# rgcgithub/regenie

Hardware: AMD Instinct MI355X
Metric: Step-1 SNPs x samples x phenos / sec (higher is better)
Workload: dtype fp4 (exact integer Gram) + i8 (exact fixed-point digit planes of the fp64 operands: G~X / G~Y, many-row predictions) + f64 (solves, level 1); 1 GPU; BASELINE configs[1]: synthetic PLINK bed 50000 samples x 100000 SNPs (100000 per GPU), 1 QT pheno, bsize 1000, 22 chromosomes, 5-fold CV, 5x5 ridge grid; `value` is the HBM-resident figure (packed genotypes generated on the device, timed region = level 0 + level 1 + LOCO rows); the complete run from files on disk is `end_to_end_from_files`; samples=50000, snps=100000, phenos=1, bsize=1000, blocks=109, parallelism=blocks sharded x1, all-gather of W, level-1 Gram tiles / ridge systems shared x1

## Files before the change

regenie_amd/build.py:

```python
from __future__ import annotations

import concurrent.futures as cf
import hashlib
import os
import shutil
import subprocess
import sys

HERE = os.path.dirname(os.path.abspath(__file__))
CSRC = os.path.join(HERE, "csrc")
LIBDIR = os.path.join(HERE, "lib")
LIB = os.path.join(LIBDIR, "librg_step1_hip.so")
SOURCES = ["rg_api.hip", "bed_prep.hip", "gram_i8.hip", "gram_fp4.hip", "assemble.hip", "chol.hip", "pred.hip", "l1.hip", "ubench.hip", "loocv.hip", "loocv_tri.hip", "l1x.hip", "l0_f64.hip", "step2_qt.hip", "step2_bt.hip", "step2_mcc.hip", "rg_group.hip", "pred_i8.hip", "xy_i8.hip", "wgram_bf16.hip", "bgen_inflate.hip", "ld_corr.hip",
           "pgen_api.cpp", "bgen_api.cpp"]
HOST_SOURCES = ["driver_common.cpp", "driver_models.cpp", "driver_inputs.cpp", "driver_step2.cpp", "driver_step2_bgen.cpp", "driver_ld.cpp", "driver_step1.cpp", "driver_main.cpp"]
FLAGS = ["--offload-arch=gfx950", "-O3", "-std=c++17", "-fPIC", "-Wall", "-Wno-unused-function",
         "-Wno-unused-variable", "-Wno-unused-value", "-Wno-unused-result", "-Wno-inline-asm"]


def _hipcc() -> str:
    for c in (shutil.which("hipcc"), "/opt/rocm/bin/hipcc"):
        if c and os.path.exists(c):
            return c
    raise RuntimeError("hipcc not found")
# ... 24 lines not shown
        with open(os.path.join(HERE, rel), "rb") as fh:
            out[rel] = hashlib.sha256(fh.read()).hexdigest()
    out["flags"] = hashlib.sha256(" ".join(FLAGS).encode()).hexdigest()
    return out


def _deps():
    return _lib_deps() + [os.path.join(HERE, "host", f) for f in HOST_SOURCES + ["driver.h", "driver_step2.h", "driver_ld.h", "fmt_g6.h"]]


def _lib_deps():
    return [os.path.join(CSRC, s) for s in SOURCES] + [
                                                      os.path.join(CSRC, "rg_internal.h"),
                                                      os.path.join(CSRC, "chol_common.h"),
                                                      os.path.join(CSRC, "chol_p128.h"),
                                                      os.path.join(CSRC, "step2_internal.h"),
                                                      os.path.join(CSRC, "pgen_reader.h"),
                                                      os.path.join(CSRC, "bgen_reader.h"),
                                                      os.path.join(CSRC, "inflate_fast.h"),
                                                      os.path.join(HERE, "..", "include", "rg_bgen.h"),
                                                      os.path.join(HERE, "..", "include", "rg_ld.h"),
                                                      os.path.join(HERE, "..", "include", "rg_pgen.h"),
                                                      os.path.join(HERE, "..", "include", "rg_step1.h"),
                                                      os.path.join(HERE, "..", "include", "rg_step2.h")]


def _write_file_digests():
    import json
    with open(os.path.join(LIBDIR, "kernel_files.json"), "w") as fh:
        json.dump(kernel_file_digests(), fh, indent=0, sort_keys=True)
# ... 60 lines not shown
```

regenie_amd/csrc/l1.hip:

```cpp
#include <algorithm>
#include <climits>
#include <cmath>
#include <cstdint>
#include <vector>
#include "rg_internal.h"

#define CT 64

struct L1Rows {
  const double* W; const double* y; const double* zero;
  int64_t Np; int L, P, p, n64;
};
__device__ __forceinline__ const double* l1_row(const L1Rows& R, int row) {
  if (row < R.L) return R.W + ((int64_t)row * R.P + R.p) * R.Np;
  if (row == R.n64) return R.y;
  return R.zero;
}

struct L1G64 {
  L1Rows R; int T, rtot, nslice, ntile, world, rank;
  double* out; int64_t slice_stride;
};
__global__ __launch_bounds__(256, 2) void k_l1_gram64(L1G64 g, SegLayout seg) {
  const int lane = threadIdx.x & 63, wave = threadIdx.x >> 6;
// ... 48 lines not shown
        mma8(a0, b0);
        if (kc + 2 < k1) load8(a0, b0, kc + 2);
        mma8(a1, b1);
      }
    }
  }
  double* O = g.out + (int64_t)sl * g.slice_stride + (int64_t)f * g.rtot * g.R.n64 + (int64_t)tr * CT * g.R.n64 + tc * CT;
#pragma unroll
  for (int m = 0; m < 4; ++m)
#pragma unroll
    for (int n = 0; n < 4; ++n)
#pragma unroll
      for (int r = 0; r < 4; ++r) O[(int64_t)(m * 16 + q + 4 * r) * g.R.n64 + n * 16 + i] = acc[m][n][r];
}

struct L1Item { int16_t mr, mc, fold, slice; };
struct L1G128 {
  L1Rows R; int rtot, nslice; const L1Item* items; double* out; int64_t slice_stride;
};
#define G128_STAGE 32768
__device__ __forceinline__ const double* l1_wrow(const L1Rows& R, int row) {
  return row < R.L ? R.W + ((int64_t)row * R.P + R.p) * R.Np : R.zero;
}
__global__ __launch_bounds__(256, 2) void k_l1_gram128(L1G128 g, SegLayout seg) {
  __shared__ __attribute__((aligned(16))) uint8_t smem[2 * G128_STAGE];
  const L1Item it = g.items[blockIdx.x];
  if (it.fold < 0) return;
  const int lane = threadIdx.x & 63, wave = __builtin_amdgcn_readfirstlane(threadIdx.x >> 6);
  const int wr = wave >> 1, wc = wave & 1;
  const int i = lane & 15, q = lane >> 4;
  const int f = it.fold, n64 = g.R.n64;
// ... 72 lines not shown
  const double* y = R.y + seg.pos_start[f];
  const int64_t n = seg.plen[f];
  double t0 = 0.0, t1 = 0.0;
  for (int64_t e = 2 * (int64_t)threadIdx.x; e < n; e += 512) {
    const double2 wv = *reinterpret_cast<const double2*>(w + e), yv = *reinterpret_cast<const double2*>(y + e);
    t0 = fma(wv.x, yv.x, t0);
    t1 = fma(wv.y, yv.y, t1);
  }
  double t = t0 + t1;
  for (int o = 32; o > 0; o >>= 1) t += __shfl_down(t, o);
  if ((threadIdx.x & 63) == 0) red[threadIdx.x >> 6] = t;
  __syncthreads();
  if (threadIdx.x == 0) out[(int64_t)f * rtot * R.n64 + (int64_t)R.n64 * R.n64 + l] = (red[0] + red[1]) + (red[2] + red[3]);
}

static std::vector<L1Item> l1_build_items(int n64, int K, int nslice, int world, int rank) {
  const int T2 = (n64 + 127) / 128, S = 4, TS = (T2 + S - 1) / S;
  std::vector<std::vector<L1Item>> xl(8);
  int gi = 0;
  for (int f = 0; f < K; ++f)
    for (int sl = 0; sl < nslice; ++sl)
      for (int Mr = 0; Mr < TS; ++Mr)
        for (int Mc = 0; Mc <= Mr; ++Mc) {
          std::vector<L1Item>& dst = xl[gi % 8];
          bool any = false;
          for (int mr = Mr * S; mr < std::min(T2, (Mr + 1) * S); ++mr)
            for (int mc = Mc * S; mc < std::min(T2, (Mc + 1) * S); ++mc) {
              if (mc > mr) continue;
              if ((mr * (mr + 1) / 2 + mc) % world != rank) continue;
              dst.push_back(L1Item{(int16_t)mr, (int16_t)mc, (int16_t)f, (int16_t)sl});
              any = true;
            }
          if (any) ++gi;
        }
  size_t mx = 0;
  for (auto& v : xl) mx = std::max(mx, v.size());
  std::vector<L1Item> items(mx * 8, L1Item{0, 0, -1, 0});
  for (int x = 0; x < 8; ++x)
    for (size_t j = 0; j < xl[x].size(); ++j) items[8 * j + x] = xl[x][j];
  return items;
}

void rg_launch_fold_gram_rows(hipStream_t st, const double* G, int64_t ld, int L, int n64, int rtot, const double* zero,
                              const SegLayout& seg, double* out) {
  L1G64 g;
  g.R = L1Rows{G, zero, zero, ld, L, 1, 0, n64};
  g.T = n64 / CT; g.rtot = rtot; g.nslice = 1; g.ntile = g.T * (g.T + 1) / 2 + g.T; g.world = 1; g.rank = 0;
  g.out = out; g.slice_stride = 0;
  hipLaunchKernelGGL(k_l1_gram64, dim3((g.ntile + 3) / 4, seg.nseg), dim3(256), 0, st, g, seg);
}

__global__ void k_reduce_slices(const double* part, int64_t slice_stride, int nslice, int64_t n, double* out) {
  const int64_t e = (int64_t)blockIdx.x * blockDim.x + threadIdx.x;
  if (e >= n) return;
  double t = 0.0;
  for (int s = 0; s < nslice; ++s) t += part[(int64_t)s * slice_stride + e];
  out[e] = t;
}

__global__ void k_sum_folds(const double* fold, int64_t msz, int nfold, double* sum) {
  const int64_t e = (int64_t)blockIdx.x * blockDim.x + threadIdx.x;
  if (e >= msz) return;
  double t = 0.0;
  for (int f = 0; f < nfold; ++f) t += fold[(int64_t)f * msz + e];
  sum[e] = t;
}

__global__ __launch_bounds__(256) void k_loco(const double* pred, int nchr, int64_t N, const int32_t* chrom, int nchrom,
                                              double* out) {
  const int64_t n = (int64_t)blockIdx.x * 256 + threadIdx.x;
  if (n >= N) return;
  double tot = 0.0;
  for (int k = 0; k < nchr; ++k) tot += pred[(int64_t)k * N + n];
  for (int c = 0; c < nchrom; ++c) out[(int64_t)c * N + n] = tot;
  for (int k = 0; k < nchr; ++k) out[(int64_t)(chrom[k] - 1) * N + n] = tot - pred[(int64_t)k * N + n];
}

int rg_emit_pred(rg_ctx* ctx, hipStream_t st, const double* d_pred, int nchr, int p, double* pred_out) {
  const int64_t N = ctx->N;
  if (ctx->loco_nchrom <= 0) {
    RG_HIP(hipMemcpyAsync(pred_out + (int64_t)p * nchr * N, d_pred, sizeof(double) * (size_t)nchr * N, hipMemcpyDeviceToHost, st));
    return RG_OK;
  }
  if ((int)ctx->loco_chrom.size() != nchr) { ctx->err = "LOCO output: rg_set_loco_output was given a different number of chromosomes"; return RG_ERR_ARG; }
  const int nchrom = ctx->loco_nchrom;
  double* d_out = (double*)rg_ws(ctx, 11, sizeof(double) * (size_t)nchrom * N + sizeof(int32_t) * (size_t)nchr + 64);
  if (!d_out) { ctx->err = "LOCO output: out of device memory"; return RG_ERR_HIP; }
  int32_t* d_chr = reinterpret_cast<int32_t*>(d_out + (size_t)nchrom * N);
  RG_HIP(hipMemcpyAsync(d_chr, ctx->loco_chrom.data(), sizeof(int32_t) * nchr, hipMemcpyHostToDevice, st));
  hipLaunchKernelGGL(k_loco, dim3((unsigned)((N + 255) / 256)), dim3(256), 0, st, d_pred, nchr, N, d_chr, nchrom, d_out);
  RG_HIP(hipMemcpyAsync(pred_out + (int64_t)p * nchrom * N, d_out, sizeof(double) * (size_t)nchrom * N, hipMemcpyDeviceToHost, st));
  return RG_OK;
}

__global__ __launch_bounds__(256) void k_tiles_pack(double* fold, int64_t msz, int T, int n64, double* packed, int unpack) {
  const int t = blockIdx.x, f = blockIdx.y;
  int tr = (int)((sqrtf(8.0f * t + 1.0f) - 1.0f) * 0.5f);
  while ((tr + 1) * (tr + 2) / 2 <= t) ++tr;
  while (tr * (tr + 1) / 2 > t) --tr;
  int tc = t - tr * (tr + 1) / 2;
  if (tr >= T) { tc = t - T * (T + 1) / 2; tr = T; }
  double* src = fold + (int64_t)f * msz + (int64_t)tr * CT * n64 + tc * CT;
  double* pk = packed + ((int64_t)f * gridDim.x + t) * (CT * CT);
  for (int e = threadIdx.x; e < CT * CT; e += 256) {
    const int r = e >> 6, c = e & 63;
    if (unpack) src[(int64_t)r * n64 + c] = pk[e];
    else pk[e] = src[(int64_t)r * n64 + c];
  }
}

#define R1MAX 8
#define L1_CT 256
__global__ __launch_bounds__(256) void k_l1_cv(L1Rows R, const double* alpha , int R1,
                                               const int32_t* chunk_seg, const int64_t* chunk_pos,
                                               const int64_t* chunk_len, double* part) {
  __shared__ double sA[L1_CT][R1MAX];
  __shared__ double sred[4][R1MAX * 3 + 2];
  const int ch = blockIdx.x;
  const int f = chunk_seg[ch];
  const int64_t p0 = chunk_pos[ch], plen = chunk_len[ch];
  double tot[R1MAX * 3 + 2];
#pragma unroll
  for (int t = 0; t < R1MAX * 3 + 2; ++t) tot[t] = 0.0;
  for (int64_t sub = 0; sub < plen; sub += 256) {
    const int64_t pos = p0 + sub + threadIdx.x;
    const bool live = sub + threadIdx.x < plen;
    double acc[R1MAX];
#pragma unroll
    for (int j = 0; j < R1MAX; ++j) acc[j] = 0.0;
    for (int c0 = 0; c0 < R.L; c0 += L1_CT) {
      __syncthreads();
      for (int j = 0; j < R1MAX; ++j) {
        const int col = c0 + threadIdx.x;
        sA[threadIdx.x][j] = (j < R1 && col < R.L)
            ? alpha[((int64_t)f * R1 + j) * R.n64 + col] : 0.0;
      }
      __syncthreads();
      if (live) {
        const int cn = min(L1_CT, R.L - c0);
        const double* w = R.W + ((int64_t)c0 * R.P + R.p) * R.Np + pos;
        for (int c = 0; c < cn; ++c) {
          const double x = w[(int64_t)c * R.P * R.Np];
#pragma unroll
          for (int j = 0; j < R1MAX; ++j) acc[j] = fma(x, sA[c][j], acc[j]);
        }
      }
    }
    if (live) {
      const double y = R.y[pos];
#pragma unroll
      for (int j = 0; j < R1MAX; ++j) {
        tot[3 * j] += acc[j];
        tot[3 * j + 1] = fma(acc[j], acc[j], tot[3 * j + 1]);
        tot[3 * j + 2] = fma(acc[j], y, tot[3 * j + 2]);
      }
      tot[R1MAX * 3] += y;
      tot[R1MAX * 3 + 1] = fma(y, y, tot[R1MAX * 3 + 1]);
    }
  }
#pragma unroll
  for (int t = 0; t < R1MAX * 3 + 2; ++t) {
    double x = tot[t];
    for (int o = 32; o > 0; o >>= 1) x += __shfl_down(x, o);
    if ((threadIdx.x & 63) == 0) sred[threadIdx.x >> 6][t] = x;
  }
  __syncthreads();
  if (threadIdx.x < R1MAX * 3 + 2)
    part[(int64_t)ch * (R1MAX * 3 + 2) + threadIdx.x] =
        (sred[0][threadIdx.x] + sred[1][threadIdx.x]) + (sred[2][threadIdx.x] + sred[3][threadIdx.x]);
}

__global__ __launch_bounds__(256) void k_l1_pred(L1Rows R, const double* alpha , int R1,
                                                 int best, const int32_t* chunk_seg,
                                                 const int64_t* chunk_pos, const int64_t* chunk_len,
                                                 const int32_t* chr_col0 , int nchr,
                                                 const int32_t* cidx, int64_t N, double* pred) {
  extern __shared__ double sAl[];
  const int ch = blockIdx.x;
  const int f = chunk_seg[ch];
  const int64_t p0 = chunk_pos[ch], plen = chunk_len[ch];
  const double* al = alpha + ((int64_t)f * R1 + best) * R.n64;
  for (int c = threadIdx.x; c < R.L; c += 256) sAl[c] = al[c];
  __syncthreads();
  for (int64_t sub = 0; sub < plen; sub += 256) {
    const int64_t pos = p0 + sub + threadIdx.x;
    if (sub + threadIdx.x >= plen) continue;
    const int32_t n = cidx[pos];
    if (n < 0) continue;
    for (int c = 0; c < nchr; ++c) {
      double acc = 0.0;
      const double* w = R.W + ((int64_t)chr_col0[c] * R.P + R.p) * R.Np + pos;
      const int nn = chr_col0[c + 1] - chr_col0[c];
      for (int t = 0; t < nn; ++t) acc = fma(w[(int64_t)t * R.P * R.Np], sAl[chr_col0[c] + t], acc);
      pred[(int64_t)c * N + n] = acc;
    }
  }
}

int rg_l1_qt_impl(rg_ctx* ctx, int R1, const double* tau, int nchr, const int32_t* cols_per_chr,
                  double* cumsum_out, int32_t* best_out, double* pred_out) {
  if (!ctx->have_problem || !(ctx->d_W || ctx->v_W)) { ctx->err = "rg_l1_qt: no level-0 predictors"; return RG_ERR_STATE; }
  if (R1 < 1 || R1 > R1MAX) { ctx->err = "rg_l1_qt: n_ridge_l1 must be in [1,8]"; return RG_ERR_ARG; }
  if (ctx->loocv) { ctx->err = "rg_l1_qt: the problem was set up for LOOCV (use rg_l1_qt_loocv)"; return RG_ERR_STATE; }
  hipStream_t st = ctx->stream;
  const int L = ctx->B_total * ctx->R0, K = ctx->K;
  if (!ctx->v_W && ctx->w_nb != ctx->B_total) { ctx->err = "rg_l1_qt: W holds a block range only (rg_set_block_range): level 1 needs the exchanged view"; return RG_ERR_STATE; }
  const double* Wv = ctx->v_W ? ctx->v_W : ctx->d_W;
  const int Pv = ctx->v_W ? ctx->v_np : ctx->P, P = ctx->v_np, p0v = ctx->v_p0;
  int ltot = 0;
  std::vector<int32_t> col0(nchr + 1, 0);
  for (int c = 0; c < nchr; ++c) { col0[c + 1] = col0[c] + cols_per_chr[c]; }
  ltot = col0[nchr];
  if (ltot != L) { ctx->err = "rg_l1_qt: cols_per_chr does not sum to n_blocks*R0"; return RG_ERR_ARG; }
  const int n64 = (int)rg_round_up(L, CT), rtot = n64 + CT, T = n64 / CT;
  const int64_t msz = (int64_t)rtot * n64;
  const int nsys = K * R1;
  const int nch = ctx->n_c256;
  const int NPART = R1MAX * 3 + 2;
  const int world = ctx->coll_world, rank = ctx->coll_rank;
  const bool multi = ctx->coll_allreduce != nullptr;
  const int b0 = multi ? (int)((int64_t)nsys * rank / world) : 0;
  const int b1 = multi ? (int)((int64_t)nsys * (rank + 1) / world) : nsys;
  const int nloc = b1 - b0;
  const int ntile = T * (T + 1) / 2 + T;
  int64_t min_nch = INT64_MAX;
  for (int f = 0; f < K; ++f) min_nch = std::min(min_nch, ctx->seg.plen[f] / 64);
  const int T2 = (n64 + 127) / 128, ntile2 = T2 * (T2 + 1) / 2;
  int nslice = (int)std::min<int64_t>(16, std::max<int64_t>(1, (3072 + (int64_t)ntile2 * K - 1) / ((int64_t)ntile2 * K)));
  nslice = (int)std::max<int64_t>(1, std::min<int64_t>(nslice, min_nch / 2));

  double *d_fold = nullptr, *d_part = nullptr, *d_sum = nullptr, *d_wk = nullptr, *d_dinv = nullptr, *d_tau = nullptr,
         *d_cvp = nullptr, *d_pred = nullptr, *d_alpha = nullptr, *d_pack = nullptr;
  int32_t* d_col0 = nullptr;
#define L1_WS(var, slot, type, count)                                                   \
  var = (type*)rg_ws(ctx, slot, sizeof(type) * (size_t)(count));                        \
  if (!var) { ctx->err = "rg_l1_qt: out of device memory"; return RG_ERR_HIP; }
  L1_WS(d_fold, 0, double, msz * K)
  if (nslice > 1) { L1_WS(d_part, 1, double, msz * K * nslice) }
  L1_WS(d_sum, 2, double, msz)
  L1_WS(d_wk, 3, double, msz * std::max(1, nloc))
  L1_WS(d_dinv, 4, double, rg_chol_ws_doubles((size_t)std::max(1, nloc), n64))
  L1_WS(d_tau, 5, double, R1)
  L1_WS(d_cvp, 6, double, (size_t)nch * NPART)
  L1_WS(d_pred, 7, double, (size_t)nchr * ctx->N)
  L1_WS(d_alpha, 8, double, (size_t)nsys * n64)
  L1_WS(d_col0, 9, int32_t, nchr + 1)
  if (multi) { L1_WS(d_pack, 10, double, (size_t)ntile * K * CT * CT) }
  L1Item* d_items = nullptr;
  const std::vector<L1Item> items = l1_build_items(n64, K, nslice, multi ? world : 1, multi ? rank : 0);
  L1_WS(d_items, 12, L1Item, items.size())
  RG_HIP(hipMemcpyAsync(d_items, items.data(), sizeof(L1Item) * items.size(), hipMemcpyHostToDevice, st));
  RG_HIP(hipStreamSynchronize(st));
#undef L1_WS
  RG_HIP(hipMemcpyAsync(d_col0, col0.data(), sizeof(int32_t) * (nchr + 1), hipMemcpyHostToDevice, st));
  std::vector<double> hpart((size_t)nch * NPART);
  int rc = RG_OK;
  auto lap = [&](double* slot, hipEvent_t e0, hipEvent_t e1) {
    if (!ctx->timing) return;
    hipEventRecord(e1, st); hipEventSynchronize(e1);
    float ms; hipEventElapsedTime(&ms, e0, e1); *slot += ms;
    hipEventRecord(e0, st);
  };

  for (int p = 0; p < P && rc == RG_OK; ++p) {
    const int pg = p0v + p, pw = ctx->v_W ? p : pg;
    L1Rows R{Wv, ctx->d_V + (int64_t)(ctx->C + pg) * ctx->Np, ctx->d_zero, ctx->Np, L, Pv, pw, n64};
    hipEvent_t e0 = ctx->ev0, e1 = ctx->ev1;
    if (ctx->timing) hipEventRecord(e0, st);
    double* gout = nslice > 1 ? d_part : d_fold;
    hipMemsetAsync(gout, 0, sizeof(double) * msz * K * nslice, st);
    L1G128 g{R, rtot, nslice, d_items, gout, msz * K};
    hipLaunchKernelGGL(k_l1_gram128, dim3((unsigned)items.size()), dim3(256), 0, st, g, ctx->seg);
    if (nslice > 1)
      hipLaunchKernelGGL(k_reduce_slices, dim3((unsigned)((msz * K + 255) / 256)), dim3(256), 0, st, d_part, msz * K,
                         nslice, msz * K, d_fold);
    hipLaunchKernelGGL(k_l1_wty, dim3(L, K), dim3(256), 0, st, R, ctx->seg, rtot, multi ? world : 1, multi ? rank : 0, d_fold);
    if (multi) {
      hipLaunchKernelGGL(k_tiles_pack, dim3(ntile, K), dim3(256), 0, st, d_fold, msz, T, n64, d_pack, 0);
      RG_HIP(hipStreamSynchronize(st));
      if (ctx->coll_allreduce(ctx->coll_user, d_pack, (int64_t)ntile * K * CT * CT) != 0) { ctx->err = "rg_l1_qt: all-reduce callback failed"; rc = RG_ERR_STATE; break; }
      hipLaunchKernelGGL(k_tiles_pack, dim3(ntile, K), dim3(256), 0, st, d_fold, msz, T, n64, d_pack, 1);
    }
    hipLaunchKernelGGL(k_sum_folds, dim3((unsigned)((msz + 255) / 256)), dim3(256), 0, st, d_fold, msz, K, d_sum);
    lap(&ctx->tm.ms_l1_gram, e0, e1);
    hipMemcpyAsync(d_tau, tau + (int64_t)p * R1, sizeof(double) * R1, hipMemcpyHostToDevice, st);
    hipMemsetAsync(d_alpha, 0, sizeof(double) * (size_t)nsys * n64, st);
    if (nloc > 0) {
      rg_launch_chol_solve_formed_x(st, d_sum, 0, d_fold, msz, K, d_tau, R1, nullptr, L, 1, d_wk, msz, n64, CT, 1,
                                    d_dinv, ctx->d_info + 1, &ctx->tm.n_chol_launches, 1, nullptr, 0, 0, 1, b0, nloc);
      RG_HIP(hipMemcpy2DAsync(d_alpha + (int64_t)b0 * n64, sizeof(double) * n64, d_wk + (int64_t)n64 * n64,
                              sizeof(double) * msz, sizeof(double) * n64, nloc, hipMemcpyDeviceToDevice, st));
    }
    if (multi) {
      RG_HIP(hipStreamSynchronize(st));
      if (ctx->coll_allreduce(ctx->coll_user, d_alpha, (int64_t)nsys * n64) != 0) { ctx->err = "rg_l1_qt: all-reduce callback failed"; rc = RG_ERR_STATE; break; }
    }
    lap(&ctx->tm.ms_l1_chol, e0, e1);
    hipLaunchKernelGGL(k_l1_cv, dim3(nch), dim3(256), 0, st, R, d_alpha, R1, ctx->d_c256_seg,
                       ctx->d_c256_pos, ctx->d_c256_len, d_cvp);
    RG_HIP(hipMemcpyAsync(hpart.data(), d_cvp, sizeof(double) * hpart.size(), hipMemcpyDeviceToHost, st));
    RG_HIP(hipStreamSynchronize(st));
    double* cs = cumsum_out + (int64_t)p * 5 * R1;
    for (int t = 0; t < 5 * R1; ++t) cs[t] = 0.0;
    double sy = 0.0, sy2 = 0.0;
    for (int ch = 0; ch < nch; ++ch) {
      const double* q = hpart.data() + (size_t)ch * NPART;
      for (int j = 0; j < R1; ++j) {
        cs[0 * R1 + j] += q[3 * j];
        cs[2 * R1 + j] += q[3 * j + 1];
        cs[4 * R1 + j] += q[3 * j + 2];
      }
      sy += q[R1MAX * 3];
      sy2 += q[R1MAX * 3 + 1];
    }
    for (int j = 0; j < R1; ++j) { cs[1 * R1 + j] = sy; cs[3 * R1 + j] = sy2; }
    int best = 0; double minv = 1e10;
    for (int j = 0; j < R1; ++j) {
      const double perf = (cs[2 * R1 + j] + cs[3 * R1 + j] - 2 * cs[4 * R1 + j]) / ctx->neff[pg];
      if (perf < minv) { best = j; minv = perf; }
    }
    best_out[p] = best;
    hipMemsetAsync(d_pred, 0, sizeof(double) * (size_t)nchr * ctx->N, st);
    hipLaunchKernelGGL(k_l1_pred, dim3(nch), dim3(256), sizeof(double) * L, st, R, d_alpha, R1, best,
                       ctx->d_c256_seg, ctx->d_c256_pos, ctx->d_c256_len, d_col0, nchr,
                       ctx->d_cidx, ctx->N, d_pred);
    if ((rc = rg_emit_pred(ctx, st, d_pred, nchr, p, pred_out))) break;
    RG_HIP(hipStreamSynchronize(st));
    if (ctx->timing) { hipEventRecord(e1, st); hipEventSynchronize(e1); float ms; hipEventElapsedTime(&ms, e0, e1); ctx->tm.ms_l1_pred += ms; }
    int32_t info[2] = {0, 0};
    RG_HIP(hipMemcpy(info, ctx->d_info, sizeof(info), hipMemcpyDeviceToHost));
    if (info[1]) { ctx->err = "level 1 ridge system is not positive definite"; rc = RG_ERR_NOT_SPD; }
  }
  return rc;
}
```

regenie_amd/csrc/rg_api.hip:

```cpp
#include <algorithm>
#include <cstdlib>
#include <cstring>
#include <chrono>
#include "rg_internal.h"

namespace {

template <class T>
int dev_alloc(rg_ctx* ctx, T** p, size_t n) {
  if (*p) { hipFree(*p); *p = nullptr; }
  if (n == 0) n = 1;
  RG_HIP(hipMalloc((void**)p, n * sizeof(T)));
  return RG_OK;
}
template <class T>
int dev_upload(rg_ctx* ctx, T** p, const std::vector<T>& v) {
  int rc = dev_alloc(ctx, p, v.size());
  if (rc) return rc;
  if (!v.empty()) RG_HIP(hipMemcpy(*p, v.data(), v.size() * sizeof(T), hipMemcpyHostToDevice));
  return RG_OK;
}

void free_all(rg_ctx* c) {
  void* ptrs[] = {c->d_cidx, c->d_act, c->d_V, c->d_maskp, c->d_Q, c->d_XtY, c->d_lambda, c->d_neff,
// ... 44 lines not shown
  hipEventCreate(&c->ev0);
  hipEventCreate(&c->ev1);
  *out = c;
  return RG_OK;
}

void rg_destroy(rg_ctx* c) {
  if (!c) return;
  hipSetDevice(c->device);
  if (c->twin) { rg_destroy(c->twin); c->twin = nullptr; }
  if (c->ev_ingest) hipEventDestroy(c->ev_ingest);
  if (c->ev_tw_fork) hipEventDestroy(c->ev_tw_fork);
  if (c->ev_tw_join) hipEventDestroy(c->ev_tw_join);
  hipStreamSynchronize(c->stream);
  free_all(c);
  if (c->ev0) hipEventDestroy(c->ev0);
  if (c->ev1) hipEventDestroy(c->ev1);
  if (c->ev_fork) {
    hipEventDestroy(c->ev_fork);
    for (int k = 0; k < 3; ++k) { hipStreamSynchronize(c->st_part[k]); hipStreamDestroy(c->st_part[k]); hipEventDestroy(c->ev_part[k]); }
  }
  if (c->st_stage) { hipStreamSynchronize(c->st_stage); hipStreamDestroy(c->st_stage); }
  if (c->own_stream) hipStreamDestroy(c->stream);
  delete c;
}

const char* rg_last_error(const rg_ctx* c) { return c ? c->err.c_str() : "null context"; }

int rg_set_problem(rg_ctx* ctx, const rg_problem* p) {
  if (!ctx || !p) return RG_ERR_ARG;
// ... 820 lines not shown
```

regenie_amd/csrc/rg_internal.h:

```cpp
#pragma once
#include <hip/hip_runtime.h>
#include <stdint.h>
#include <functional>
#include <string>
#include <vector>

#include "../../include/rg_step1.h"

#define RG_MAX_SEG 32
#define RG_TILE_G 128
#define RG_TILE_C 64

typedef int v4i __attribute__((ext_vector_type(4)));
typedef int v16i __attribute__((ext_vector_type(16)));
typedef double v4d __attribute__((ext_vector_type(4)));

static inline int64_t rg_round_up(int64_t x, int64_t m) { return (x + m - 1) / m * m; }
static inline size_t rg_chol_ws_doubles(size_t batch, int n64) {
  const size_t T = (size_t)n64 / 64;
  return batch * (T + (T + 3) / 4 * 10) * 4096;
}

struct SegLayout {
  int32_t nseg;
// ... 117 lines not shown
  rg_allreduce_fn coll_allreduce = nullptr;
  void* coll_user = nullptr;

  rg_ctx* twin = nullptr;
  int n_pipe = 1;
  bool is_child = false;
  hipEvent_t ev_tw_fork = nullptr, ev_tw_join = nullptr;
  bool join_pending = false;
  int pipe_rr = 0;

  hipEvent_t ev_ingest = nullptr;
  bool ingest_pending = false;

  void* ws_ptr[16] = {};
  size_t ws_bytes[16] = {};

  void* f64_ptr[10] = {};
  size_t f64_bytes[10] = {};

  bool timing = false;
  rg_timing tm{};
  hipEvent_t ev0 = nullptr, ev1 = nullptr;
};

static inline double* rg_w_base(const rg_ctx* c) { return c->d_W ? c->d_W - (int64_t)c->w_b0 * c->R0 * c->P * c->Np : nullptr; }

static inline void* rg_ws(rg_ctx* ctx, int slot, size_t bytes) {
  if (bytes == 0) bytes = 8;
  if (ctx->ws_bytes[slot] < bytes) {
    if (ctx->ws_ptr[slot]) hipFree(ctx->ws_ptr[slot]);
// ... 108 lines not shown
  int64_t Np, pk_ld, pk_blk_stride;
  const uint8_t* pk; const double* mu; const double* sc; const double* Bm; const double* V;
  const double* maskp; const double* neff; const int32_t* bs; const int32_t* blockid;
  const double* wk; double* gt; double* W;
  int64_t gt_pos0 = 0, gt_len = 0;
};
size_t rg_loocv_tri_ws_doubles(int nblk, int n64, int P, int R0);
int rg_l0_loocv_tri(rg_ctx* ctx, hipStream_t st, const LoocvArgs& la, int max_bs, const double* d_sum, int rtot, double* ws, double* zt,
                    int64_t chunk, const std::function<void(int64_t, int64_t)>& gt_chunk);
void rg_launch_decode_gt(hipStream_t st, const LoocvArgs& a);
void rg_launch_l0_loocv(hipStream_t st, const LoocvArgs& a, double* part0, double* part1, int nchunk);
void rg_launch_fold_gram_rows(hipStream_t st, const double* G, int64_t ld, int L, int n64, int rtot, const double* zero,
                              const SegLayout& seg, double* out);
int rg_l0_blocks_f64_impl(rg_ctx* ctx, int nblk, const int32_t* block_ids, const int32_t* bs, const double* const* rows,
                          int64_t row_stride, int mem_kind);
int rg_emit_pred(rg_ctx* ctx, hipStream_t st, const double* d_pred, int nchr, int p, double* pred_out);
struct L1Args;
int rg_l1_qt_impl(rg_ctx* ctx, int R1, const double* tau, int nchr, const int32_t* cols_per_chr,
                  double* cumsum_out, int32_t* best_out, double* pred_out);
#define RG_WGRAM_FP16 1
#define RG_WGRAM_BF16X3 2
int rg_launch_wgram_bf16(rg_ctx* ctx, hipStream_t st, const double* W, int64_t Np, int L, int P, int p, int n64, const double* wv, double* sw, int nchain,
                         const int32_t* d_chainmap, const int32_t* h_chainmap, int nslot, int excl_own, double* part, int64_t out_stride,
                         int max_slices, int fmt);
int rg_l1_qt_loocv_impl(rg_ctx* ctx, int R1, const double* tau, int nchr, const int32_t* cols_per_chr,
                        double* cumsum_out, int32_t* best_out, double* pred_out);
int rg_l1_cox_impl(rg_ctx* ctx, int pheno, int R1, const double* time, const double* event, const double* offset, const rg_cox_options* opt,
                   int nchr, const int32_t* cols_per_chr, double* tau_out, double* deviance_out, int32_t* converged_out, int32_t* best_out,
                   double* pred_out);
int rg_l1_bt_impl(rg_ctx* ctx, int R1, const double* tau, const double* yraw, const double* offset,
                  const rg_bt_options* opt, int nchr, const int32_t* cols_per_chr, double* cumsum_out,
// ... 2 lines not shown
```

Baseline: 166.6 billion SNP*sample*pheno/s.

## Fuse level-1 CV and prediction, select best on device, cache staged tables

Result: faster. 170.1 billion SNP*sample*pheno/s, median of 6 (+2.1%).

```diff
diff --git a/regenie_amd/build.py b/regenie_amd/build.py
--- a/regenie_amd/build.py
+++ b/regenie_amd/build.py
@@ -62,6 +62,7 @@
                                                       os.path.join(CSRC, "rg_internal.h"),
                                                       os.path.join(CSRC, "chol_common.h"),
                                                       os.path.join(CSRC, "chol_p128.h"),
+                                                      os.path.join(CSRC, "l1_stage.h"),
                                                       os.path.join(CSRC, "step2_internal.h"),
                                                       os.path.join(CSRC, "pgen_reader.h"),
                                                       os.path.join(CSRC, "bgen_reader.h"),
diff --git a/regenie_amd/csrc/l1.hip b/regenie_amd/csrc/l1.hip
--- a/regenie_amd/csrc/l1.hip
+++ b/regenie_amd/csrc/l1.hip
@@ -86,7 +86,6 @@
       for (int r = 0; r < 4; ++r) O[(int64_t)(m * 16 + q + 4 * r) * g.R.n64 + n * 16 + i] = acc[m][n][r];
 }
 
-struct L1Item { int16_t mr, mc, fold, slice; };
 struct L1G128 {
   L1Rows R; int rtot, nslice; const L1Item* items; double* out; int64_t slice_stride;
 };
@@ -189,33 +188,6 @@
   if (threadIdx.x == 0) out[(int64_t)f * rtot * R.n64 + (int64_t)R.n64 * R.n64 + l] = (red[0] + red[1]) + (red[2] + red[3]);
 }
 
-static std::vector<L1Item> l1_build_items(int n64, int K, int nslice, int world, int rank) {
-  const int T2 = (n64 + 127) / 128, S = 4, TS = (T2 + S - 1) / S;
-  std::vector<std::vector<L1Item>> xl(8);
-  int gi = 0;
-  for (int f = 0; f < K; ++f)
-    for (int sl = 0; sl < nslice; ++sl)
-      for (int Mr = 0; Mr < TS; ++Mr)
-        for (int Mc = 0; Mc <= Mr; ++Mc) {
-          std::vector<L1Item>& dst = xl[gi % 8];
-          bool any = false;
-          for (int mr = Mr * S; mr < std::min(T2, (Mr + 1) * S); ++mr)
-            for (int mc = Mc * S; mc < std::min(T2, (Mc + 1) * S); ++mc) {
-              if (mc > mr) continue;
-              if ((mr * (mr + 1) / 2 + mc) % world != rank) continue;
-              dst.push_back(L1Item{(int16_t)mr, (int16_t)mc, (int16_t)f, (int16_t)sl});
-              any = true;
-            }
-          if (any) ++gi;
-        }
-  size_t mx = 0;
-  for (auto& v : xl) mx = std::max(mx, v.size());
-  std::vector<L1Item> items(mx * 8, L1Item{0, 0, -1, 0});
-  for (int x = 0; x < 8; ++x)
-    for (size_t j = 0; j < xl[x].size(); ++j) items[8 * j + x] = xl[x][j];
-  return items;
-}
-
 void rg_launch_fold_gram_rows(hipStream_t st, const double* G, int64_t ld, int L, int n64, int rtot, const double* zero,
                               const SegLayout& seg, double* out) {
   L1G64 g;
@@ -242,18 +214,40 @@
 }
 
 __global__ __launch_bounds__(256) void k_loco(const double* pred, int nchr, int64_t N, const int32_t* chrom, int nchrom,
-                                              double* out) {
+                                              double* out, const int32_t* sel) {
   const int64_t n = (int64_t)blockIdx.x * 256 + threadIdx.x;
   if (n >= N) return;
+  if (sel) pred += (int64_t)sel[0] * nchr * N;
   double tot = 0.0;
   for (int k = 0; k < nchr; ++k) tot += pred[(int64_t)k * N + n];
   for (int c = 0; c < nchrom; ++c) out[(int64_t)c * N + n] = tot;
   for (int k = 0; k < nchr; ++k) out[(int64_t)(chrom[k] - 1) * N + n] = tot - pred[(int64_t)k * N + n];
 }
 
-int rg_emit_pred(rg_ctx* ctx, hipStream_t st, const double* d_pred, int nchr, int p, double* pred_out) {
+__global__ __launch_bounds__(256) void k_pick_set(const double* cand, int64_t n, const int32_t* sel, double* out) {
+  const int64_t e = (int64_t)blockIdx.x * 256 + threadIdx.x;
+  if (e < n) out[e] = cand[(int64_t)sel[0] * n + e];
+}
+
+L1StageAlloc rg_l1_stage_alloc() {
+  L1StageAlloc a;
+  a.host_alloc = [](size_t b) -> void* { void* p = nullptr; if (hipHostMalloc(&p, b, hipHostMallocDefault) != hipSuccess) { (void)hipGetLastError(); return nullptr; } return p; };
+  a.host_free = [](void* p) { hipHostFree(p); };
+  a.dev_alloc = [](size_t b) -> void* { void* p = nullptr; if (hipMalloc(&p, b) != hipSuccess) { (void)hipGetLastError(); return nullptr; } return p; };
+  a.dev_free = [](void* p) { hipFree(p); };
+  return a;
+}
+
+int rg_emit_pred(rg_ctx* ctx, hipStream_t st, const double* d_pred, int nchr, int p, double* pred_out, const int32_t* d_sel,
+                 const int32_t* d_chrom) {
   const int64_t N = ctx->N;
   if (ctx->loco_nchrom <= 0) {
+    if (d_sel) {
+      double* d_one = (double*)rg_ws(ctx, 11, sizeof(double) * (size_t)nchr * N);
+      if (!d_one) { ctx->err = "level-1 output: out of device memory"; return RG_ERR_HIP; }
+      hipLaunchKernelGGL(k_pick_set, dim3((unsigned)(((int64_t)nchr * N + 255) / 256)), dim3(256), 0, st, d_pred, (int64_t)nchr * N, d_sel, d_one);
+      d_pred = d_one;
+    }
     RG_HIP(hipMemcpyAsync(pred_out + (int64_t)p * nchr * N, d_pred, sizeof(double) * (size_t)nchr * N, hipMemcpyDeviceToHost, st));
     return RG_OK;
   }
@@ -261,9 +255,13 @@
   const int nchrom = ctx->loco_nchrom;
   double* d_out = (double*)rg_ws(ctx, 11, sizeof(double) * (size_t)nchrom * N + sizeof(int32_t) * (size_t)nchr + 64);
   if (!d_out) { ctx->err = "LOCO output: out of device memory"; return RG_ERR_HIP; }
-  int32_t* d_chr = reinterpret_cast<int32_t*>(d_out + (size_t)nchrom * N);
-  RG_HIP(hipMemcpyAsync(d_chr, ctx->loco_chrom.data(), sizeof(int32_t) * nchr, hipMemcpyHostToDevice, st));
-  hipLaunchKernelGGL(k_loco, dim3((unsigned)((N + 255) / 256)), dim3(256), 0, st, d_pred, nchr, N, d_chr, nchrom, d_out);
+  const int32_t* d_chr = d_chrom;
+  if (!d_chr) {
+    int32_t* up = reinterpret_cast<int32_t*>(d_out + (size_t)nchrom * N);
+    RG_HIP(hipMemcpyAsync(up, ctx->loco_chrom.data(), sizeof(int32_t) * nchr, hipMemcpyHostToDevice, st));
+    d_chr = up;
+  }
+  hipLaunchKernelGGL(k_loco, dim3((unsigned)((N + 255) / 256)), dim3(256), 0, st, d_pred, nchr, N, d_chr, nchrom, d_out, d_sel);
   RG_HIP(hipMemcpyAsync(pred_out + (int64_t)p * nchrom * N, d_out, sizeof(double) * (size_t)nchrom * N, hipMemcpyDeviceToHost, st));
   return RG_OK;
 }
@@ -284,47 +282,83 @@
   }
 }
 
-#define R1MAX 8
+#define R1MAX L1_R1MAX
 #define L1_CT 256
-__global__ __launch_bounds__(256) void k_l1_cv(L1Rows R, const double* alpha , int R1,
-                                               const int32_t* chunk_seg, const int64_t* chunk_pos,
-                                               const int64_t* chunk_len, double* part) {
+#define L1_U 16
+template <int R1T>
+__global__ __launch_bounds__(256) void k_l1_cvpred(L1Rows R, const double* alpha , const int32_t* chunk_seg,
+                                                   const int64_t* chunk_pos, const int64_t* chunk_len,
+                                                   const int32_t* chr_col0 , int nchr, const int32_t* cidx, int64_t N,
+                                                   double* part, double* cand) {
   __shared__ double sA[L1_CT][R1MAX];
-  __shared__ double sred[4][R1MAX * 3 + 2];
+  __shared__ double sred[4][L1_NPART];
   const int ch = blockIdx.x;
   const int f = chunk_seg[ch];
   const int64_t p0 = chunk_pos[ch], plen = chunk_len[ch];
-  double tot[R1MAX * 3 + 2];
-#pragma unroll
-  for (int t = 0; t < R1MAX * 3 + 2; ++t) tot[t] = 0.0;
+  const int64_t stride = (int64_t)R.P * R.Np;
+  double tot[L1_NPART];
+#pragma unroll
+  for (int t = 0; t < L1_NPART; ++t) tot[t] = 0.0;
   for (int64_t sub = 0; sub < plen; sub += 256) {
-    const int64_t pos = p0 + sub + threadIdx.x;
     const bool live = sub + threadIdx.x < plen;
-    double acc[R1MAX];
-#pragma unroll
-    for (int j = 0; j < R1MAX; ++j) acc[j] = 0.0;
+    const int64_t pos = live ? p0 + sub + threadIdx.x : p0;
+    const int32_t n = live ? cidx[pos] : -1;
+    double acc[R1T], pc[R1T];
+#pragma unroll
+    for (int j = 0; j < R1T; ++j) { acc[j] = 0.0; pc[j] = 0.0; }
+    int cc = 0, cend = chr_col0[1];
+    auto flush = [&]() {
+#pragma unroll
+      for (int j = 0; j < R1T; ++j) {
+        if (n >= 0) cand[((int64_t)j * nchr + cc) * N + n] = pc[j];
+        pc[j] = 0.0;
+      }
+    };
     for (int c0 = 0; c0 < R.L; c0 += L1_CT) {
       __syncthreads();
-      for (int j = 0; j < R1MAX; ++j) {
+#pragma unroll
+      for (int j = 0; j < R1T; ++j) {
         const int col = c0 + threadIdx.x;
-        sA[threadIdx.x][j] = (j < R1 && col < R.L)
-            ? alpha[((int64_t)f * R1 + j) * R.n64 + col] : 0.0;
+        sA[threadIdx.x][j] = col < R.L ? alpha[((int64_t)f * R1T + j) * R.n64 + col] : 0.0;
       }
       __syncthreads();
-      if (live) {
-        const int cn = min(L1_CT, R.L - c0);
-        const double* w = R.W + ((int64_t)c0 * R.P + R.p) * R.Np + pos;
-        for (int c = 0; c < cn; ++c) {
-          const double x = w[(int64_t)c * R.P * R.Np];
-#pragma unroll
-          for (int j = 0; j < R1MAX; ++j) acc[j] = fma(x, sA[c][j], acc[j]);
+      const int cn = min(L1_CT, R.L - c0);
+      const double* w = R.W + ((int64_t)c0 * R.P + R.p) * R.Np + pos;
+      auto use1 = [&](double x, int c) {
+        while (c0 + c == cend && cc + 1 < nchr) { flush(); ++cc; cend = chr_col0[cc + 1]; }
+#pragma unroll
+        for (int j = 0; j < R1T; ++j) {
+          acc[j] = fma(x, sA[c][j], acc[j]);
+          pc[j] = fma(x, sA[c][j], pc[j]);
+        }
+      };
+      auto ld = [&](double (&x)[L1_U], int c) {
+#pragma unroll
+        for (int u = 0; u < L1_U; ++u) x[u] = w[(int64_t)(c + u) * stride];
+      };
+      auto use = [&](const double (&x)[L1_U], int c) {
+#pragma unroll
+        for (int u = 0; u < L1_U; ++u) use1(x[u], c + u);
+      };
+      const int cfull = cn / L1_U * L1_U;
+      double xa[L1_U], xb[L1_U];
+      if (cfull > 0) ld(xa, 0);
+      for (int c = 0; c < cfull; c += 2 * L1_U) {
+        const bool more = c + L1_U < cfull;
+        if (more) ld(xb, c + L1_U);
+        use(xa, c);
+        if (more) {
+          if (c + 2 * L1_U < cfull) ld(xa, c + 2 * L1_U);
+          use(xb, c + L1_U);
         }
       }
-    }
+      for (int c = cfull; c < cn; ++c) use1(w[(int64_t)c * stride], c);
+    }
+    while (cc < nchr) { flush(); ++cc; }
     if (live) {
       const double y = R.y[pos];
 #pragma unroll
-      for (int j = 0; j < R1MAX; ++j) {
+      for (int j = 0; j < R1T; ++j) {
         tot[3 * j] += acc[j];
         tot[3 * j + 1] = fma(acc[j], acc[j], tot[3 * j + 1]);
         tot[3 * j + 2] = fma(acc[j], y, tot[3 * j + 2]);
@@ -334,42 +368,49 @@
     }
   }
 #pragma unroll
-  for (int t = 0; t < R1MAX * 3 + 2; ++t) {
+  for (int t = 0; t < L1_NPART; ++t) {
     double x = tot[t];
     for (int o = 32; o > 0; o >>= 1) x += __shfl_down(x, o);
     if ((threadIdx.x & 63) == 0) sred[threadIdx.x >> 6][t] = x;
   }
   __syncthreads();
-  if (threadIdx.x < R1MAX * 3 + 2)
-    part[(int64_t)ch * (R1MAX * 3 + 2) + threadIdx.x] =
+  if (threadIdx.x < L1_NPART)
+    part[(int64_t)ch * L1_NPART + threadIdx.x] =
         (sred[0][threadIdx.x] + sred[1][threadIdx.x]) + (sred[2][threadIdx.x] + sred[3][threadIdx.x]);
 }
 
-__global__ __launch_bounds__(256) void k_l1_pred(L1Rows R, const double* alpha , int R1,
-                                                 int best, const int32_t* chunk_seg,
-                                                 const int64_t* chunk_pos, const int64_t* chunk_len,
-                                                 const int32_t* chr_col0 , int nchr,
-                                                 const int32_t* cidx, int64_t N, double* pred) {
-  extern __shared__ double sAl[];
-  const int ch = blockIdx.x;
-  const int f = chunk_seg[ch];
-  const int64_t p0 = chunk_pos[ch], plen = chunk_len[ch];
-  const double* al = alpha + ((int64_t)f * R1 + best) * R.n64;
-  for (int c = threadIdx.x; c < R.L; c += 256) sAl[c] = al[c];
+__global__ __launch_bounds__(256) void k_l1_select(const double* part, int nch, int R1, const double* neff, const int32_t* info,
+                                                   L1Res* res) {
+  __shared__ double sp[128][L1_NPART];
+  __shared__ double stot[L1_NPART];
+  double t = 0.0;
+  for (int c0 = 0; c0 < nch; c0 += 128) {
+    const int nc = min(128, nch - c0);
+    __syncthreads();
+    for (int e = threadIdx.x; e < nc * L1_NPART; e += 256) (&sp[0][0])[e] = part[(int64_t)c0 * L1_NPART + e];
+    __syncthreads();
+    if (threadIdx.x < L1_NPART)
+      for (int c = 0; c < nc; ++c) t += sp[c][threadIdx.x];
+  }
+  if (threadIdx.x < L1_NPART) { stot[threadIdx.x] = t; res->tot[threadIdx.x] = t; }
   __syncthreads();
-  for (int64_t sub = 0; sub < plen; sub += 256) {
-    const int64_t pos = p0 + sub + threadIdx.x;
-    if (sub + threadIdx.x >= plen) continue;
-    const int32_t n = cidx[pos];
-    if (n < 0) continue;
-    for (int c = 0; c < nchr; ++c) {
-      double acc = 0.0;
-      const double* w = R.W + ((int64_t)chr_col0[c] * R.P + R.p) * R.Np + pos;
-      const int nn = chr_col0[c + 1] - chr_col0[c];
-      for (int t = 0; t < nn; ++t) acc = fma(w[(int64_t)t * R.P * R.Np], sAl[chr_col0[c] + t], acc);
-      pred[(int64_t)c * N + n] = acc;
-    }
-  }
+  if (threadIdx.x == 0) {
+    const double sy2 = stot[R1MAX * 3 + 1], ne = neff[0];
+    int best = 0; double minv = 1e10;
+    for (int j = 0; j < R1; ++j) {
+      const double perf = (stot[3 * j + 1] + sy2 - 2 * stot[3 * j + 2]) / ne;
+      if (perf < minv) { best = j; minv = perf; }
+    }
+    res->best = best;
+    res->info = info[1];
+  }
+}
+
+template <int R1T>
+static void l1_launch_cvpred(hipStream_t st, int nch, const L1Rows& R, const double* alpha, const rg_ctx* ctx, const int32_t* col0,
+                             int nchr, double* part, double* cand) {
+  hipLaunchKernelGGL(k_l1_cvpred<R1T>, dim3(nch), dim3(256), 0, st, R, alpha, ctx->d_c256_seg, ctx->d_c256_pos, ctx->d_c256_len,
+                     col0, nchr, ctx->d_cidx, ctx->N, part, cand);
 }
 
 int rg_l1_qt_impl(rg_ctx* ctx, int R1, const double* tau, int nchr, const int32_t* cols_per_chr,
@@ -382,16 +423,16 @@
   if (!ctx->v_W && ctx->w_nb != ctx->B_total) { ctx->err = "rg_l1_qt: W holds a block range only (rg_set_block_range): level 1 needs the exchanged view"; return RG_ERR_STATE; }
   const double* Wv = ctx->v_W ? ctx->v_W : ctx->d_W;
   const int Pv = ctx->v_W ? ctx->v_np : ctx->P, P = ctx->v_np, p0v = ctx->v_p0;
-  int ltot = 0;
-  std::vector<int32_t> col0(nchr + 1, 0);
-  for (int c = 0; c < nchr; ++c) { col0[c + 1] = col0[c] + cols_per_chr[c]; }
-  ltot = col0[nchr];
+  int64_t ltot = 0;
+  for (int c = 0; c < nchr; ++c) {
+    if (cols_per_chr[c] < 0) { ctx->err = "rg_l1_qt: negative cols_per_chr entry"; return RG_ERR_ARG; }
+    ltot += cols_per_chr[c];
+  }
   if (ltot != L) { ctx->err = "rg_l1_qt: cols_per_chr does not sum to n_blocks*R0"; return RG_ERR_ARG; }
   const int n64 = (int)rg_round_up(L, CT), rtot = n64 + CT, T = n64 / CT;
   const int64_t msz = (int64_t)rtot * n64;
   const int nsys = K * R1;
   const int nch = ctx->n_c256;
-  const int NPART = R1MAX * 3 + 2;
   const int world = ctx->coll_world, rank = ctx->coll_rank;
   const bool multi = ctx->coll_allreduce != nullptr;
   const int b0 = multi ? (int)((int64_t)nsys * rank / world) : 0;
@@ -404,9 +445,8 @@
   int nslice = (int)std::min<int64_t>(16, std::max<int64_t>(1, (3072 + (int64_t)ntile2 * K - 1) / ((int64_t)ntile2 * K)));
   nslice = (int)std::max<int64_t>(1, std::min<int64_t>(nslice, min_nch / 2));
 
-  double *d_fold = nullptr, *d_part = nullptr, *d_sum = nullptr, *d_wk = nullptr, *d_dinv = nullptr, *d_tau = nullptr,
-         *d_cvp = nullptr, *d_pred = nullptr, *d_alpha = nullptr, *d_pack = nullptr;
-  int32_t* d_col0 = nullptr;
+  double *d_fold = nullptr, *d_part = nullptr, *d_sum = nullptr, *d_wk = nullptr, *d_dinv = nullptr,
+         *d_cvp = nullptr, *d_cand = nullptr, *d_alpha = nullptr, *d_pack = nullptr;
 #define L1_WS(var, slot, type, count)                                                   \
   var = (type*)rg_ws(ctx, slot, sizeof(type) * (size_t)(count));                        \
   if (!var) { ctx->err = "rg_l1_qt: out of device memory"; return RG_ERR_HIP; }
@@ -415,20 +455,26 @@
   L1_WS(d_sum, 2, double, msz)
   L1_WS(d_wk, 3, double, msz * std::max(1, nloc))
   L1_WS(d_dinv, 4, double, rg_chol_ws_doubles((size_t)std::max(1, nloc), n64))
-  L1_WS(d_tau, 5, double, R1)
-  L1_WS(d_cvp, 6, double, (size_t)nch * NPART)
-  L1_WS(d_pred, 7, double, (size_t)nchr * ctx->N)
+  L1_WS(d_cvp, 6, double, (size_t)nch * L1_NPART)
+  L1_WS(d_cand, 7, double, (size_t)R1 * nchr * ctx->N)
   L1_WS(d_alpha, 8, double, (size_t)nsys * n64)
-  L1_WS(d_col0, 9, int32_t, nchr + 1)
   if (multi) { L1_WS(d_pack, 10, double, (size_t)ntile * K * CT * CT) }
-  L1Item* d_items = nullptr;
-  const std::vector<L1Item> items = l1_build_items(n64, K, nslice, multi ? world : 1, multi ? rank : 0);
-  L1_WS(d_items, 12, L1Item, items.size())
-  RG_HIP(hipMemcpyAsync(d_items, items.data(), sizeof(L1Item) * items.size(), hipMemcpyHostToDevice, st));
-  RG_HIP(hipStreamSynchronize(st));
 #undef L1_WS
-  RG_HIP(hipMemcpyAsync(d_col0, col0.data(), sizeof(int32_t) * (nchr + 1), hipMemcpyHostToDevice, st));
-  std::vector<double> hpart((size_t)nch * NPART);
+  L1Stage& S = ctx->l1st;
+  const bool loco = ctx->loco_nchrom > 0;
+  int upload = 0;
+  if (l1_stage_prepare(S, rg_l1_stage_alloc(), n64, K, nslice, multi ? world : 1, multi ? rank : 0, nchr, cols_per_chr,
+                       loco ? (int)ctx->loco_chrom.size() : 0, ctx->loco_chrom.data(), P, R1, &upload)) {
+    ctx->err = "rg_l1_qt: out of page-locked host or device memory for the level-1 tables"; return RG_ERR_HIP;
+  }
+  if (upload) RG_HIP(hipMemcpyAsync(S.dev, S.host, S.table_bytes, hipMemcpyHostToDevice, st));
+  memcpy(S.h<double>(S.off_tau), tau, sizeof(double) * (size_t)P * R1);
+  RG_HIP(hipMemcpyAsync(S.d<double>(S.off_tau), S.h<double>(S.off_tau), sizeof(double) * (size_t)P * R1, hipMemcpyHostToDevice, st));
+  const L1Item* d_items = S.d<L1Item>(S.off_items);
+  const int32_t* d_col0 = S.d<int32_t>(S.off_col0);
+  const int32_t* d_chrom = loco ? S.d<int32_t>(S.off_chrom) : nullptr;
+  L1Res* d_res = S.d<L1Res>(S.off_res);
+  L1Res* h_res = S.h<L1Res>(S.off_res);
   int rc = RG_OK;
   auto lap = [&](double* slot, hipEvent_t e0, hipEvent_t e1) {
     if (!ctx->timing) return;
@@ -437,15 +483,17 @@
     hipEventRecord(e0, st);
   };
 
+  int pdone = 0;
   for (int p = 0; p < P && rc == RG_OK; ++p) {
     const int pg = p0v + p, pw = ctx->v_W ? p : pg;
     L1Rows R{Wv, ctx->d_V + (int64_t)(ctx->C + pg) * ctx->Np, ctx->d_zero, ctx->Np, L, Pv, pw, n64};
+    const double* d_tau = S.d<double>(S.off_tau) + (int64_t)p * R1;
     hipEvent_t e0 = ctx->ev0, e1 = ctx->ev1;
     if (ctx->timing) hipEventRecord(e0, st);
     double* gout = nslice > 1 ? d_part : d_fold;
     hipMemsetAsync(gout, 0, sizeof(double) * msz * K * nslice, st);
     L1G128 g{R, rtot, nslice, d_items, gout, msz * K};
-    hipLaunchKernelGGL(k_l1_gram128, dim3((unsigned)items.size()), dim3(256), 0, st, g, ctx->seg);
+    hipLaunchKernelGGL(k_l1_gram128, dim3((unsigned)S.n_items), dim3(256), 0, st, g, ctx->seg);
     if (nslice > 1)
       hipLaunchKernelGGL(k_reduce_slices, dim3((unsigned)((msz * K + 255) / 256)), dim3(256), 0, st, d_part, msz * K,
                          nslice, msz * K, d_fold);
@@ -458,7 +506,6 @@
     }
     hipLaunchKernelGGL(k_sum_folds, dim3((unsigned)((msz + 255) / 256)), dim3(256), 0, st, d_fold, msz, K, d_sum);
     lap(&ctx->tm.ms_l1_gram, e0, e1);
-    hipMemcpyAsync(d_tau, tau + (int64_t)p * R1, sizeof(double) * R1, hipMemcpyHostToDevice, st);
     hipMemsetAsync(d_alpha, 0, sizeof(double) * (size_t)nsys * n64, st);
     if (nloc > 0) {
       rg_launch_chol_solve_formed_x(st, d_sum, 0, d_fold, msz, K, d_tau, R1, nullptr, L, 1, d_wk, msz, n64, CT, 1,
@@ -471,40 +518,35 @@
       if (ctx->coll_allreduce(ctx->coll_user, d_alpha, (int64_t)nsys * n64) != 0) { ctx->err = "rg_l1_qt: all-reduce callback failed"; rc = RG_ERR_STATE; break; }
     }
     lap(&ctx->tm.ms_l1_chol, e0, e1);
-    hipLaunchKernelGGL(k_l1_cv, dim3(nch), dim3(256), 0, st, R, d_alpha, R1, ctx->d_c256_seg,
-                       ctx->d_c256_pos, ctx->d_c256_len, d_cvp);
-    RG_HIP(hipMemcpyAsync(hpart.data(), d_cvp, sizeof(double) * hpart.size(), hipMemcpyDeviceToHost, st));
-    RG_HIP(hipStreamSynchronize(st));
+    switch (R1) {
+      case 1: l1_launch_cvpred<1>(st, nch, R, d_alpha, ctx, d_col0, nchr, d_cvp, d_cand); break;
+      case 2: l1_launch_cvpred<2>(st, nch, R, d_alpha, ctx, d_col0, nchr, d_cvp, d_cand); break;
+      case 3: l1_launch_cvpred<3>(st, nch, R, d_alpha, ctx, d_col0, nchr, d_cvp, d_cand); break;
+      case 4: l1_launch_cvpred<4>(st, nch, R, d_alpha, ctx, d_col0, nchr, d_cvp, d_cand); break;
+      case 5: l1_launch_cvpred<5>(st, nch, R, d_alpha, ctx, d_col0, nchr, d_cvp, d_cand); break;
+      case 6: l1_launch_cvpred<6>(st, nch, R, d_alpha, ctx, d_col0, nchr, d_cvp, d_cand); break;
+      case 7: l1_launch_cvpred<7>(st, nch, R, d_alpha, ctx, d_col0, nchr, d_cvp, d_cand); break;
+      default: l1_launch_cvpred<8>(st, nch, R, d_alpha, ctx, d_col0, nchr, d_cvp, d_cand); break;
+    }
+    hipLaunchKernelGGL(k_l1_select, dim3(1), dim3(256), 0, st, d_cvp, nch, R1, ctx->d_neff + pg, ctx->d_info, d_res + p);
+    if ((rc = rg_emit_pred(ctx, st, d_cand, nchr, p, pred_out, &d_res[p].best, d_chrom))) break;
+    RG_HIP(hipMemcpyAsync(h_res + p, d_res + p, sizeof(L1Res), hipMemcpyDeviceToHost, st));
+    ++pdone;
+    if (ctx->timing) { hipEventRecord(e1, st); hipEventSynchronize(e1); float ms; hipEventElapsedTime(&ms, e0, e1); ctx->tm.ms_l1_pred += ms; }
+  }
+  RG_HIP(hipStreamSynchronize(st));
+  for (int p = 0; p < pdone; ++p) {
+    const L1Res& r = h_res[p];
     double* cs = cumsum_out + (int64_t)p * 5 * R1;
-    for (int t = 0; t < 5 * R1; ++t) cs[t] = 0.0;
-    double sy = 0.0, sy2 = 0.0;
-    for (int ch = 0; ch < nch; ++ch) {
-      const double* q = hpart.data() + (size_t)ch * NPART;
-      for (int j = 0; j < R1; ++j) {
-        cs[0 * R1 + j] += q[3 * j];
-        cs[2 * R1 + j] += q[3 * j + 1];
-        cs[4 * R1 + j] += q[3 * j + 2];
-      }
-      sy += q[R1MAX * 3];
-      sy2 += q[R1MAX * 3 + 1];
-    }
-    for (int j = 0; j < R1; ++j) { cs[1 * R1 + j] = sy; cs[3 * R1 + j] = sy2; }
-    int best = 0; double minv = 1e10;
     for (int j = 0; j < R1; ++j) {
-      const double perf = (cs[2 * R1 + j] + cs[3 * R1 + j] - 2 * cs[4 * R1 + j]) / ctx->neff[pg];
-      if (perf < minv) { best = j; minv = perf; }
-    }
-    best_out[p] = best;
-    hipMemsetAsync(d_pred, 0, sizeof(double) * (size_t)nchr * ctx->N, st);
-    hipLaunchKernelGGL(k_l1_pred, dim3(nch), dim3(256), sizeof(double) * L, st, R, d_alpha, R1, best,
-                       ctx->d_c256_seg, ctx->d_c256_pos, ctx->d_c256_len, d_col0, nchr,
-                       ctx->d_cidx, ctx->N, d_pred);
-    if ((rc = rg_emit_pred(ctx, st, d_pred, nchr, p, pred_out))) break;
-    RG_HIP(hipStreamSynchronize(st));
-    if (ctx->timing) { hipEventRecord(e1, st); hipEventSynchronize(e1); float ms; hipEventElapsedTime(&ms, e0, e1); ctx->tm.ms_l1_pred += ms; }
-    int32_t info[2] = {0, 0};
-    RG_HIP(hipMemcpy(info, ctx->d_info, sizeof(info), hipMemcpyDeviceToHost));
-    if (info[1]) { ctx->err = "level 1 ridge system is not positive definite"; rc = RG_ERR_NOT_SPD; }
+      cs[0 * R1 + j] = r.tot[3 * j];
+      cs[1 * R1 + j] = r.tot[R1MAX * 3];
+      cs[2 * R1 + j] = r.tot[3 * j + 1];
+      cs[3 * R1 + j] = r.tot[R1MAX * 3 + 1];
+      cs[4 * R1 + j] = r.tot[3 * j + 2];
+    }
+    best_out[p] = r.best;
+    if (r.info && rc == RG_OK) { ctx->err = "level 1 ridge system is not positive definite"; rc = RG_ERR_NOT_SPD; }
   }
   return rc;
 }
diff --git a/regenie_amd/csrc/l1_stage.h b/regenie_amd/csrc/l1_stage.h
--- /dev/null
+++ b/regenie_amd/csrc/l1_stage.h
@@ -0,0 +1,112 @@
+#pragma once
+#include <stdint.h>
+#include <stddef.h>
+#include <string.h>
+#include <algorithm>
+#include <vector>
+
+#define L1_R1MAX 8
+#define L1_NPART (L1_R1MAX * 3 + 2)
+
+struct L1Item { int16_t mr, mc, fold, slice; };
+
+struct L1Res {
+  double tot[L1_NPART];
+  int32_t best, info;
+};
+
+static inline std::vector<L1Item> l1_build_items(int n64, int K, int nslice, int world, int rank) {
+  const int T2 = (n64 + 127) / 128, S = 4, TS = (T2 + S - 1) / S;
+  std::vector<std::vector<L1Item>> xl(8);
+  int gi = 0;
+  for (int f = 0; f < K; ++f)
+    for (int sl = 0; sl < nslice; ++sl)
+      for (int Mr = 0; Mr < TS; ++Mr)
+        for (int Mc = 0; Mc <= Mr; ++Mc) {
+          std::vector<L1Item>& dst = xl[gi % 8];
+          bool any = false;
+          for (int mr = Mr * S; mr < std::min(T2, (Mr + 1) * S); ++mr)
+            for (int mc = Mc * S; mc < std::min(T2, (Mc + 1) * S); ++mc) {
+              if (mc > mr) continue;
+              if ((mr * (mr + 1) / 2 + mc) % world != rank) continue;
+              dst.push_back(L1Item{(int16_t)mr, (int16_t)mc, (int16_t)f, (int16_t)sl});
+              any = true;
+            }
+          if (any) ++gi;
+        }
+  size_t mx = 0;
+  for (auto& v : xl) mx = std::max(mx, v.size());
+  std::vector<L1Item> items(mx * 8, L1Item{0, 0, -1, 0});
+  for (int x = 0; x < 8; ++x)
+    for (size_t j = 0; j < xl[x].size(); ++j) items[8 * j + x] = xl[x][j];
+  return items;
+}
+
+struct L1StageAlloc {
+  void* (*host_alloc)(size_t bytes);
+  void (*host_free)(void* p);
+  void* (*dev_alloc)(size_t bytes);
+  void (*dev_free)(void* p);
+};
+
+struct L1Stage {
+  int n64 = 0, K = 0, nslice = 0, world = 0, rank = 0, P = 0, R1 = 0;
+  std::vector<int32_t> cols, chrom;
+  uint8_t* host = nullptr;
+  uint8_t* dev = nullptr;
+  size_t capacity = 0;
+  size_t n_items = 0, off_items = 0, off_col0 = 0, off_chrom = 0, off_tau = 0, off_res = 0, table_bytes = 0, total = 0;
+
+  template <class T> T* h(size_t off) const { return reinterpret_cast<T*>(host + off); }
+  template <class T> T* d(size_t off) const { return reinterpret_cast<T*>(dev + off); }
+};
+
+static inline size_t l1_stage_align(size_t x) { return (x + 63) / 64 * 64; }
+
+static inline void l1_stage_release(L1Stage& s, const L1StageAlloc& a) {
+  if (s.host) a.host_free(s.host);
+  if (s.dev) a.dev_free(s.dev);
+  s = L1Stage();
+}
+
+static inline int l1_stage_prepare(L1Stage& s, const L1StageAlloc& a, int n64, int K, int nslice, int world, int rank, int nchr,
+                                   const int32_t* cols_per_chr, int nloco, const int32_t* loco_chrom, int P, int R1, int* upload) {
+  *upload = 0;
+  const bool same = s.host && s.n64 == n64 && s.K == K && s.nslice == nslice && s.world == world && s.rank == rank && s.P == P &&
+                    s.R1 == R1 && (int)s.cols.size() == nchr && std::equal(s.cols.begin(), s.cols.end(), cols_per_chr) &&
+                    (int)s.chrom.size() == nloco && std::equal(s.chrom.begin(), s.chrom.end(), loco_chrom);
+  if (same) return 0;
+  const std::vector<L1Item> items = l1_build_items(n64, K, nslice, world, rank);
+  size_t off = 0;
+  const size_t off_items = off;  off = l1_stage_align(off + sizeof(L1Item) * items.size());
+  const size_t off_col0 = off;   off = l1_stage_align(off + sizeof(int32_t) * ((size_t)nchr + 1));
+  const size_t off_chrom = off;  off = l1_stage_align(off + sizeof(int32_t) * (size_t)std::max(1, nloco));
+  const size_t table_bytes = off;
+  const size_t off_tau = off;    off = l1_stage_align(off + sizeof(double) * (size_t)P * R1);
+  const size_t off_res = off;    off = l1_stage_align(off + sizeof(L1Res) * (size_t)P);
+  if (off > s.capacity) {
+    uint8_t* nh = (uint8_t*)a.host_alloc(off);
+    uint8_t* nd = nh ? (uint8_t*)a.dev_alloc(off) : nullptr;
+    if (!nh || !nd) {
+      if (nh) a.host_free(nh);
+      l1_stage_release(s, a);
+      return -1;
+    }
+    if (s.host) a.host_free(s.host);
+    if (s.dev) a.dev_free(s.dev);
+    s.host = nh; s.dev = nd; s.capacity = off;
+  }
+  s.n64 = n64; s.K = K; s.nslice = nslice; s.world = world; s.rank = rank; s.P = P; s.R1 = R1;
+  s.cols.assign(cols_per_chr, cols_per_chr + nchr);
+  s.chrom.assign(loco_chrom, loco_chrom + nloco);
+  s.n_items = items.size(); s.off_items = off_items; s.off_col0 = off_col0; s.off_chrom = off_chrom; s.off_tau = off_tau;
+  s.off_res = off_res; s.table_bytes = table_bytes; s.total = off;
+  memset(s.host, 0, s.total);
+  if (!items.empty()) memcpy(s.h<L1Item>(off_items), items.data(), sizeof(L1Item) * items.size());
+  int32_t* col0 = s.h<int32_t>(off_col0);
+  col0[0] = 0;
+  for (int c = 0; c < nchr; ++c) col0[c + 1] = col0[c] + cols_per_chr[c];
+  if (nloco > 0) memcpy(s.h<int32_t>(off_chrom), loco_chrom, sizeof(int32_t) * (size_t)nloco);
+  *upload = 1;
+  return 0;
+}
diff --git a/regenie_amd/csrc/rg_api.hip b/regenie_amd/csrc/rg_api.hip
--- a/regenie_amd/csrc/rg_api.hip
+++ b/regenie_amd/csrc/rg_api.hip
@@ -82,6 +82,7 @@
   if (c->ev_tw_join) hipEventDestroy(c->ev_tw_join);
   hipStreamSynchronize(c->stream);
   free_all(c);
+  l1_stage_release(c->l1st, rg_l1_stage_alloc());
   if (c->ev0) hipEventDestroy(c->ev0);
   if (c->ev1) hipEventDestroy(c->ev1);
   if (c->ev_fork) {
diff --git a/regenie_amd/csrc/rg_internal.h b/regenie_amd/csrc/rg_internal.h
--- a/regenie_amd/csrc/rg_internal.h
+++ b/regenie_amd/csrc/rg_internal.h
@@ -6,6 +6,7 @@
 #include <vector>
 
 #include "../../include/rg_step1.h"
+#include "l1_stage.h"
 
 #define RG_MAX_SEG 32
 #define RG_TILE_G 128
@@ -155,6 +156,7 @@
 
   void* ws_ptr[16] = {};
   size_t ws_bytes[16] = {};
+  L1Stage l1st;
 
   void* f64_ptr[10] = {};
   size_t f64_bytes[10] = {};
@@ -293,7 +295,9 @@
                               const SegLayout& seg, double* out);
 int rg_l0_blocks_f64_impl(rg_ctx* ctx, int nblk, const int32_t* block_ids, const int32_t* bs, const double* const* rows,
                           int64_t row_stride, int mem_kind);
-int rg_emit_pred(rg_ctx* ctx, hipStream_t st, const double* d_pred, int nchr, int p, double* pred_out);
+int rg_emit_pred(rg_ctx* ctx, hipStream_t st, const double* d_pred, int nchr, int p, double* pred_out, const int32_t* d_sel = nullptr,
+                 const int32_t* d_chrom = nullptr);
+L1StageAlloc rg_l1_stage_alloc();
 struct L1Args;
 int rg_l1_qt_impl(rg_ctx* ctx, int R1, const double* tau, int nchr, const int32_t* cols_per_chr,
                   double* cumsum_out, int32_t* best_out, double* pred_out);
```
